# Meng-333/FastDiffSR

Measured on AMD Instinct MI355X. Metric: 256x256 SR images/sec at T=20, higher is better.
Workload: dtype f16x3; 1 GPU; x4 64->256, batch=16/GPU, T=20, random-init FastDiffSR UNet (inner 64, mults 1-2-4-4), 256x256, conv arithmetic f16x3 (BASELINE configs[1]); batch_per_gpu=16, global_batch=16, noise=drawn in the loop by the engine (Philox4x32-10), hipgraph=False, parallelism=dp1 (independent batches, weights broadcast once)

## Files before the change

### fastdiffsr_amd/_lib.py

```python
import ctypes as C
import os

from .build import LIB

FDSR_MAX_MULTS = 8
FDSR_SAMPLE_GRAPH = 1
FDSR_METRIC_FIELDS = 8
FDSR_SSIM_UNIFORM7, FDSR_SSIM_GAUSS11 = 1, 2
PRECISIONS = {'f32': 0, 'f16x3': 1, 'bf16': 2, 'f16': 3}


class FdsrConfig(C.Structure):
    _fields_ = [('in_channel', C.c_int32), ('out_channel', C.c_int32), ('inner_channel', C.c_int32),
                ('norm_groups', C.c_int32), ('n_mults', C.c_int32), ('channel_mults', C.c_int32 * FDSR_MAX_MULTS),
                ('res_blocks', C.c_int32), ('dropout', C.c_float), ('image_size', C.c_int32), ('variant', C.c_int32),
                ('n_attn_res', C.c_int32), ('attn_res', C.c_int32 * FDSR_MAX_MULTS)]


class FdsrSchedule(C.Structure):
    _fields_ = [('n_timestep', C.c_int32), ('noise_level', C.POINTER(C.c_float)), ('sqrt_recip', C.POINTER(C.c_float)),
                ('sqrt_recipm1', C.POINTER(C.c_float)), ('coef1', C.POINTER(C.c_float)), ('coef2', C.POINTER(C.c_float)),
                ('sigma', C.POINTER(C.c_float))]


# ... 15 lines not shown
class FdsrError(RuntimeError):
    def __init__(self, code, msg):
        super().__init__(f'libfdsr_hip error {code}: {msg}')
        self.code = code


class FdsrSaturated(FdsrError):
    """f16x3: a raw convolution input left the f16 range (FDSR_E_SATURATED): the call's output is not fp32-grade."""


FDSR_E_SATURATED = -6

K32 = {'F16X3': 1, 'BF16': 2, 'RIDER_16ROW': 4, 'SMALL_GRID_2ROW': 8, 'UP2': 16, 'SMALL_WG_F16X3': 32, 'SMALL_WG_RIDER_F16X3': 64,
       'SMALL_WG_BF16': 128, 'SMALL_WG_RIDER_BF16': 512, 'RIDER_FIRST_8WAVE': 1024}
K32_DEFAULT = 1 | 2 | 8 | 16 | 32 | 64 | 128 | 1024
STRIP = {'BF16_64': 1, 'F16X3_64': 2, 'BF16_ONE_WG': 4, 'BF16_CAT64': 8, 'BF16_RIDER': 16, 'BF16_CAT128': 32, 'BF16_COUT128': 64}
STRIP_DEFAULT = 1 | 2 | 8 | 16 | 64
STRIP_ALL = 127


def bit_names(table, value):
    return '|'.join(n for n, b in table.items() if value & b) or '0'


_lib = None

SYMBOLS = {
    'fdsr_create': (C.c_int, [C.POINTER(FdsrConfig), C.POINTER(C.c_void_p)]),
    'fdsr_destroy': (None, [C.c_void_p]),
    'fdsr_last_error': (C.c_char_p, [C.c_void_p]),
    'fdsr_version': (C.c_char_p, []),
    'fdsr_num_weights': (C.c_int, [C.c_void_p]),
    'fdsr_weight_info': (C.c_int, [C.c_void_p, C.c_int, C.c_char_p, C.c_int, C.POINTER(C.c_int64), C.POINTER(C.c_int),
# ... 120 lines not shown
```

### fastdiffsr_amd/csrc/fdsr_conv_strip.hip

```cpp
#include "fdsr_kernels.h"
#include "fdsr_act_io.h"

#include <type_traits>

namespace fdsr {

typedef float s_f32x4 __attribute__((ext_vector_type(4)));
typedef unsigned s_u32x4 __attribute__((ext_vector_type(4)));
typedef _Float16 s_h8 __attribute__((ext_vector_type(8)));
typedef __bf16 s_b8 __attribute__((ext_vector_type(8)));

template <int I, int N, class F>
__device__ __forceinline__ void static_for(F&& f) {
  if constexpr (I < N) {
    f(std::integral_constant<int, I>{});
    static_for<I + 1, N>(f);
  }
}

__device__ __forceinline__ float silu_s(float v) { return v * __builtin_amdgcn_rcpf(1.0f + __expf(-v)); }

#ifndef STRIP_XS
#define STRIP_XS 4
#endif
#ifndef STRIP_XS1
#define STRIP_XS1 4
#endif
#ifndef STRIP_DIAG
#define STRIP_DIAG 0
#endif
#ifndef STRIP_FENCE3
#define STRIP_FENCE3 1
#endif

template <int PREC, int C0_, int C1_, int CR0_, int CR1_, int NPH>
struct StripCfg {
  static constexpr int NP = PREC == PREC_F16X3 ? 2 : 1;
  static constexpr int ESZ = prec_is16(PREC) ? 2 : 4;
  static constexpr int WNP = PREC == PREC_BF16 ? 1 : 2;
  static constexpr int C0 = C0_, C1 = C1_, CIN = C0_ + C1_, KCH = CIN / 32, SW = 16 * NPH, HWD = SW + 2;
  static constexpr int OPP = CIN / 8;
  static constexpr int RB = 16 * OPP * NP;
  static constexpr int SLOT_BYTES = HWD * RB;
  static constexpr int NP0 = C0_ / 32, NP1 = C1_ / 32, NPM = NP0 + NP1;
  static constexpr int NF = 3 * KCH * NPH;
  static constexpr int CR0 = CR0_, CR1 = CR1_, CR = CR0_ + CR1_, KCR = CR / 32;
  static constexpr int RRB = CR * 2;
  static constexpr int RSLOT_BYTES = SW * RRB;
  static constexpr int NR0 = CR0_ / 32, NR1 = CR1_ / 32, NPR = NR0 + NR1;
  static constexpr int NFR = KCR * NPH;
  static constexpr int NT = NF + NFR;
  static constexpr int RSLOT_OFF = 2 * SLOT_BYTES;
  static constexpr int GTAB_OFF = RSLOT_OFF + 2 * RSLOT_BYTES;
  static constexpr int OSZ = prec_is16(PREC) ? 2 : 4;
  static constexpr int PB = 64 * OSZ;
  static constexpr int UPP = PB / 16;
  static constexpr int TILE_BYTES = SW * PB;
  static constexpr int OUT_OFF = GTAB_OFF + 64 * OPP;
  static constexpr int RES_OFF = OUT_OFF + 2 * TILE_BYTES;
  static constexpr int NIT = SW * PB / 16 / 256;
  static_assert(NPH == 4, "a staging pass = 32 channels of a 64-pixel row");
  static_assert(C0_ % 32 == 0 && C1_ % 32 == 0 && CR0_ % 32 == 0 && CR1_ % 32 == 0 && C0_ > 0, "whole 32-channel chunks");
  static_assert(256 % (C0_ / 8) == 0 && (C1_ == 0 || 256 % (C1_ / 8) == 0) && (CR0_ == 0 || 256 % (CR0_ / 8) == 0) &&
                (CR1_ == 0 || 256 % (CR1_ / 8) == 0), "a thread keeps one oct index per tensor");
  static_assert(RB == 128 || RB == 256 || RB == 384 || RB == 512, "swizzles below are verified for these pixel strides");
  static_assert(CR == 0 || (prec_is16(PREC) && (RRB == 256 || RRB == 384)), "riders: the 2-byte modes (f16: launched only while the rider and the main conv share one weight scale, conv_strip_ok)");
  static_assert(NIT >= 1 && NIT <= 4 && 256 % UPP == 0, "row-tile map");
  static_assert(SLOT_BYTES + 16 * (NPH - 1) * RB < 65536 && RSLOT_BYTES < 65536, "fragment offsets must fit the ds_read immediate");
  static constexpr int NITEMS = NIT + 5 * NPM + (C1_ ? 2 : 1) + NPR + 1;
  static constexpr int slot_of(int j) { return NPH + (j * (NT - NPH)) / NITEMS; }
  static constexpr int first_item(int f) {
    int j = 0;
    while (j < NITEMS && slot_of(j) < f) ++j;
    return j;
  }
};

template <int RB>
__device__ __forceinline__ int strip_swz(int px) {
  return (RB == 128 || RB == 384) ? 2 * ((px >> 1) & 3) : 2 * (px & 7);
}

template <int PREC> struct StripRaw;
template <> struct StripRaw<PREC_BF16> {
  uint4 v;
// ... 38 lines not shown
  unsigned v;
  __device__ __forceinline__ void load(const unsigned char* ptr) { v = *reinterpret_cast<const unsigned*>(ptr); }
  __device__ __forceinline__ void pair(float& a, float& b) const {
    typedef _Float16 h2t __attribute__((ext_vector_type(2)));
    const h2t h = __builtin_bit_cast(h2t, v);
    a = (float)h[0];
    b = (float)h[1];
  }
};
template <> struct StripRawPair<PREC_F16X3> {
  float2 v;
  __device__ __forceinline__ void load(const unsigned char* ptr) { v = *reinterpret_cast<const float2*>(ptr); }
  __device__ __forceinline__ void pair(float& a, float& b) const { a = v.x; b = v.y; }
};

template <int PREC, int C0_, int C1_, int CR0_, int CR1_, int NPH, bool HAS_RES, int LB>
__global__ void __launch_bounds__(256, LB) conv_strip_kernel(const ConvParams p, const int seg_rows, const int wn_a) {
  using Cfg = StripCfg<PREC, C0_, C1_, CR0_, CR1_, NPH>;
  constexpr int NP = Cfg::NP, RB = Cfg::RB, SW = Cfg::SW, OPP = Cfg::OPP, KCH = Cfg::KCH, NF = Cfg::NF, ESZ = Cfg::ESZ;
  constexpr int NP0 = Cfg::NP0, NP1 = Cfg::NP1, NPM = Cfg::NPM, KCR = Cfg::KCR, NPR = Cfg::NPR, NR0 = Cfg::NR0, NFR = Cfg::NFR, NT = Cfg::NT;
  constexpr int RRB = Cfg::RRB;
  constexpr bool CAT = C1_ > 0, RIDER = Cfg::CR > 0;
  constexpr int XS = (LB == 1 ? STRIP_XS1 : STRIP_XS) < NF ? (LB == 1 ? STRIP_XS1 : STRIP_XS) : NF;
  using IO = ActIO<PREC>;
  typedef typename IO::Quad Quad;

  extern __shared__ __attribute__((aligned(16))) unsigned char smem_s[];
  const int tid = threadIdx.x, lane = tid & 63, w = tid >> 6, c15 = lane & 15, g = lane >> 4;
  const int H = p.Hout, W = p.Wout;

  const int stripsX = W / SW, segs = (H + seg_rows - 1) / seg_rows;
  int bid;
  {
    const int nwg = gridDim.x, b = blockIdx.x;
    const int q8 = nwg >> 3, r8 = nwg & 7, xcd = b & 7, k = b >> 3;
    bid = (xcd < r8 ? xcd * (q8 + 1) : r8 * (q8 + 1) + (xcd - r8) * q8) + k;
  }
  const int ncg = p.Cout / 64;
  const int cg = bid % ncg;
  bid /= ncg;
  const int sx = bid % stripsX;
  bid /= stripsX;
  const int seg = bid % segs;
// ... 12 lines not shown
  } else { ot[1] = 0; ppx[1] = 0; og[1] = 0; tb[1] = tb[0]; }
  constexpr unsigned PIXB[2] = {C0_ * ESZ, (CAT ? C1_ : C0_) * ESZ};
  float* gtab = reinterpret_cast<float*>(smem_s + Cfg::GTAB_OFF);
  if (tid < 4 * OPP) {
    const int c = 8 * (tid >> 2) + 2 * (tid & 3);
    const float* ps = p.gn_scale + (size_t)n * Cfg::CIN + c;
    const float* ph = p.gn_shift + (size_t)n * Cfg::CIN + c;
    *reinterpret_cast<s_f32x4*>(gtab + 4 * tid) = s_f32x4{ps[0], ps[1], ph[0], ph[1]};
  }
  __syncthreads();
  int hdst[2];
  unsigned hcol[2];
  bool hok[2];
#pragma unroll
  for (int t = 0; t < (CAT ? 2 : 1); ++t) {
    const int hside = ((lane % (2 * OPPt[t])) / OPPt[t]) & 1;
    const int hix = hside ? ox0 + SW : ox0 - 1;
    hok[t] = hix >= 0 && hix < W;
    hcol[t] = (unsigned)(hok[t] ? hix : ox0) * PIXB[t] + 2 * w * ESZ;
    const int hpx = hside ? SW + 1 : 0;
    hdst[t] = hpx * RB + 16 * (og[t] ^ strip_swz<RB>(hpx)) + 4 * w;
  }

  StripRaw<PREC> raw[3][NPM];
  StripRawPair<PREC> rawh[3][CAT ? 2 : 1];
  s_u32x4 rraw[3][RIDER ? NPR : 1];
  auto crow_in = [&](int iy) __attribute__((always_inline)) {
    const int hi = oy1 < H - 1 ? oy1 : H - 1;
    return iy < 0 ? 0 : (iy > hi ? hi : iy);
  };
  auto load_pass = [&](int iy, StripRaw<PREC>* set, int q) __attribute__((always_inline)) {
    const int t = q < NP0 ? 0 : 1, i = q < NP0 ? q : q - NP0;
    set[q].load(tb[t] + ((unsigned)(crow_in(iy) * W) + (unsigned)(ox0 + ppx[t] + i * (256 / OPPt[t]))) * PIXB[t]);
  };
  auto load_halo = [&](int iy, StripRawPair<PREC>* set, int t) __attribute__((always_inline)) {
    set[t].load(tb[t] + ((unsigned)(crow_in(iy) * W) * PIXB[t] + hcol[t]));
  };
  constexpr int OPRt[2] = {RIDER ? CR0_ / 8 : 1, RIDER && CR1_ ? CR1_ / 8 : 1};
  const unsigned char* rb[2] = {nullptr, nullptr};
  int rdst[RIDER ? NPR : 1];
  unsigned rsrc[RIDER ? NPR : 1];
  if (RIDER) {
#pragma unroll
    for (int r = 0; r < NPR; ++r) {
      const int t = r < NR0 ? 0 : 1, i = r < NR0 ? r : r - NR0;
      const int o = tid % OPRt[t], px = tid / OPRt[t] + i * (256 / OPRt[t]);
      const int ogr = (t ? CR0_ / 8 : 0) + o;
      rdst[r] = px * RRB + 16 * (ogr ^ strip_swz<RRB>(px));
// ... 49 lines not shown
      act_s0(a, b, gtab + 16 * og[t] + 4 * k, atmp);
    }
    if (stage < 0 || stage == 1) act_s1(atmp);
    if (stage < 0 || stage == 2) act_s2(atmp, d.hi[k], d.lo[PREC == PREC_F16X3 ? k : 0]);
  };
  auto write_oct = [&](const Staged& d, bool ok, unsigned char* slot, int dofs) __attribute__((always_inline)) {
    const uint4 z = {0u, 0u, 0u, 0u};
    *reinterpret_cast<uint4*>(slot + dofs) = ok ? uint4{d.hi[0], d.hi[1], d.hi[2], d.hi[3]} : z;
    if (PREC == PREC_F16X3)
      *reinterpret_cast<uint4*>(slot + (dofs ^ (16 * OPP))) = ok ? uint4{d.lo[0], d.lo[1], d.lo[2], d.lo[3]} : z;
  };
  auto stage_halo = [&](const StripRawPair<PREC>& r, int t, bool ok, unsigned char* slot, int stage) __attribute__((always_inline)) {
    if (stage <= 0) {
      float a, b;
      r.pair(a, b);
      act_s0(a, b, gtab + 16 * og[t] + 4 * w, atmp);
    }
    if (stage < 0 || stage == 1) act_s1(atmp);
    if (stage < 0 || stage == 2) {
      unsigned hi, lo = 0;
      act_s2(atmp, hi, lo);
      *reinterpret_cast<unsigned*>(slot + hdst[t]) = ok ? hi : 0u;
      if (PREC == PREC_F16X3) *reinterpret_cast<unsigned*>(slot + (hdst[t] ^ (16 * OPP))) = ok ? lo : 0u;
    }
  };
  int pdst[NPM];
#pragma unroll
  for (int q = 0; q < NPM; ++q) {
    const int t = q < NP0 ? 0 : 1, i = q < NP0 ? q : q - NP0;
    const int px = 1 + ppx[t] + i * (256 / OPPt[t]);
    pdst[q] = px * RB + 16 * (og[t] ^ strip_swz<RB>(px));
  }
  Staged stg;

  uint4 Wf[3][3][KCH][NP];
  uint4 Wr[RIDER ? KCR : 1];
  {
    const uint4* wq = reinterpret_cast<const uint4*>(p.wq);
    const int nk16 = p.Cin_pad / 16, co32 = 2 * cg + (w >> 1), cot = co32 / wn_a, wna = co32 % wn_a;
    const int wlane = 32 * (g & 1) + 16 * (w & 1) + c15;
#pragma unroll
    for (int kc = 0; kc < KCH; ++kc)
#pragma unroll
      for (int tap = 0; tap < 9; ++tap) {
        const uint4* src = wq + ((((size_t)cot * nk16 + 2 * kc + (g >> 1)) * wn_a + wna) * 9 + tap) * (Cfg::WNP * 64) + wlane;
#pragma unroll
        for (int pl = 0; pl < NP; ++pl) Wf[tap / 3][tap % 3][kc][pl] = src[pl * 64];
      }
    if (RIDER) {
      const uint4* wr = reinterpret_cast<const uint4*>(p.wq_r);
#pragma unroll
      for (int kc = 0; kc < KCR; ++kc) Wr[kc] = wr[(((size_t)cot * p.nkr + 2 * kc + (g >> 1)) * wn_a + wna) * (Cfg::WNP * 64) + wlane];
    }
  }

  int xa[3][KCH][NP];
#pragma unroll
  for (int kx = 0; kx < 3; ++kx)
#pragma unroll
    for (int kc = 0; kc < KCH; ++kc)
#pragma unroll
      for (int pl = 0; pl < NP; ++pl) {
        const int px = c15 + kx;
        xa[kx][kc][pl] = px * RB + 16 * ((pl * OPP + 4 * kc + g) ^ strip_swz<RB>(px));
      }
  int xr[RIDER ? KCR : 1];
  if (RIDER) {
#pragma unroll
    for (int kc = 0; kc < KCR; ++kc) xr[kc] = c15 * RRB + 16 * ((4 * kc + g) ^ strip_swz<RRB>(c15));
  }

  s_f32x4 acc[3][NPH];
#pragma unroll
  for (int a = 0; a < 3; ++a)
#pragma unroll
    for (int ph = 0; ph < NPH; ++ph) acc[a][ph] = s_f32x4{0.f, 0.f, 0.f, 0.f};

  const int cob = 64 * cg + 16 * w + 4 * g;
  s_f32x4 add;
  {
    const float* tembp = p.temb ? p.temb + (size_t)n * p.temb_stride + p.temb_off : p.bias;
    const float tmul = p.temb ? 1.f : 0.f;
#pragma unroll
    for (int r = 0; r < 4; ++r) {
      float a = p.bias[cob + r];
      if (RIDER) a += p.bias_r[cob + r];
      add[r] = a + tmul * tembp[cob + r];
    }
  }
  const float winv = p.w_inv_scale_dev ? *p.w_inv_scale_dev : p.w_inv_scale;
  constexpr int OSZ = Cfg::OSZ, NIT = Cfg::NIT, TILE = Cfg::TILE_BYTES;
  s_f32x4 s1 = {0.f, 0.f, 0.f, 0.f}, s2 = {0.f, 0.f, 0.f, 0.f};
  unsigned char* otile = smem_s + Cfg::OUT_OFF;
  unsigned char* rtile = smem_s + Cfg::RES_OFF;
  constexpr int PB = Cfg::PB, UPP = Cfg::UPP;
  auto tsw = [](int px) { return OSZ == 2 ? ((px >> 1) & 7) : 2 * (px & 7); };
  const int aq = OSZ == 2 ? c15 * PB + 16 * (((4 * w + g) >> 1) ^ tsw(c15)) + 8 * (g & 1)
                          : c15 * PB + 16 * ((4 * w + g) ^ tsw(c15));
  const unsigned GPB = (unsigned)p.Cout * OSZ;
  int a128[NIT];
  unsigned gofs[NIT];
#pragma unroll
  for (int i = 0; i < NIT; ++i) {
    const int px = tid / UPP + (256 / UPP) * i, u = tid % UPP;
    a128[i] = px * PB + 16 * (u ^ tsw(px));
    gofs[i] = (unsigned)((ox0 + px) * GPB + 64 * cg * OSZ + 16 * u);
  }
  const size_t img = (size_t)n * H * W * GPB;
  unsigned char* outn = reinterpret_cast<unsigned char*>(p.out) + img;
  const unsigned char* resn = reinterpret_cast<const unsigned char*>(HAS_RES ? p.res : p.out) + img;
  const uint4 z4 = {0u, 0u, 0u, 0u};
  uint4 rres0 = z4, rres1 = z4, rres2 = z4, rres3 = z4;
  auto crow = [&](int oy) __attribute__((always_inline)) { return oy < oy0 ? oy0 : (oy >= oy1 ? oy1 - 1 : oy); };
  auto load_res = [&](int oy) __attribute__((always_inline)) {
    if (HAS_RES && !(STRIP_DIAG & 1)) {
      const unsigned r0 = (unsigned)(crow(oy) * W) * GPB;
      rres0 = *reinterpret_cast<const uint4*>(resn + (r0 + gofs[0]));
      if (NIT > 1) rres1 = *reinterpret_cast<const uint4*>(resn + (r0 + gofs[NIT > 1 ? 1 : 0]));
      if (NIT > 2) rres2 = *reinterpret_cast<const uint4*>(resn + (r0 + gofs[NIT > 2 ? 2 : 0]));
// ... 13 lines not shown
    s_f32x4 v = a * winv + add;
    if (HAS_RES) v += IO::widen(*reinterpret_cast<const Quad*>(rtile + (oy & 1) * TILE + aq + 16 * PB * ph));
    unsigned char* dst = otile + (oy & 1) * TILE + aq + 16 * PB * ph;
    if (OSZ == 2) {
      *reinterpret_cast<uint2*>(dst) = pack4_16<PREC>(v);
    } else {
      *reinterpret_cast<s_f32x4*>(dst) = v;
    }
    s1 += v;
    s2 += v * v;
  };
  auto flush = [&](int oy, int i) __attribute__((always_inline)) {
    const uint4 v = *reinterpret_cast<const uint4*>(otile + (oy & 1) * TILE + a128[i]);
    if (!(STRIP_DIAG & 2)) *reinterpret_cast<uint4*>(outn + ((unsigned)(oy * W) * GPB + gofs[i])) = v;
  };

  uint4 Xf[XS][NP];
  auto mfma1 = [&](const uint4* wf, const uint4* xf, s_f32x4 c) __attribute__((always_inline)) -> s_f32x4 {
    if (PREC == PREC_F16X3) {
      c = __builtin_amdgcn_mfma_f32_16x16x32_f16(__builtin_bit_cast(s_h8, wf[0]), __builtin_bit_cast(s_h8, xf[NP - 1]), c, 0, 0, 0);
      c = __builtin_amdgcn_mfma_f32_16x16x32_f16(__builtin_bit_cast(s_h8, wf[NP - 1]), __builtin_bit_cast(s_h8, xf[0]), c, 0, 0, 0);
      return __builtin_amdgcn_mfma_f32_16x16x32_f16(__builtin_bit_cast(s_h8, wf[0]), __builtin_bit_cast(s_h8, xf[0]), c, 0, 0, 0);
    }
    return mfma16_k32<PREC>(wf[0], xf[0], c);
  };
  auto step = [&](int iy, int it, auto rot_tag, auto epi_tag, auto flush_tag) __attribute__((always_inline)) {
    constexpr int ROT = decltype(rot_tag)::value;
    constexpr bool EPI = decltype(epi_tag)::value, FLUSH = decltype(flush_tag)::value;
    constexpr int A0 = (ROT + 1) % 3, A1 = ROT, A2 = (ROT + 2) % 3;
    StripRaw<PREC>* rset = raw[(ROT + 1) % 3];
    StripRawPair<PREC>* hset = rawh[(ROT + 1) % 3];
    s_u32x4* rrs = rraw[(ROT + 1) % 3];
    unsigned char* cur = smem_s + (it & 1) * Cfg::SLOT_BYTES;
    unsigned char* nxt = smem_s + ((it & 1) ^ 1) * Cfg::SLOT_BYTES;
    unsigned char* rcur = smem_s + Cfg::RSLOT_OFF + (it & 1) * Cfg::RSLOT_BYTES;
    unsigned char* rnxt = smem_s + Cfg::RSLOT_OFF + ((it & 1) ^ 1) * Cfg::RSLOT_BYTES;
    const bool rok = iy + 1 >= 0 && iy + 1 < H;
    auto load_x = [&](auto fc) __attribute__((always_inline)) {
      constexpr int f = decltype(fc)::value;
      if constexpr (f < NF) {
        constexpr int ph = f % NPH, kc = (f / NPH) % KCH, kx = f / (NPH * KCH);
#pragma unroll
        for (int pl = 0; pl < NP; ++pl)
          Xf[f % XS][pl] = *reinterpret_cast<const uint4*>(cur + xa[kx][kc][pl] + ph * 16 * RB);
      } else if constexpr (f < NT) {
        constexpr int ph = (f - NF) % NPH, kc = (f - NF) / NPH;
        Xf[f % XS][0] = *reinterpret_cast<const uint4*>(rcur + xr[kc] + ph * 16 * RRB);
      }
    };
    auto item = [&](auto jc, auto sc) __attribute__((always_inline)) {
      constexpr int j = decltype(jc)::value, stage = decltype(sc)::value;
      constexpr int J1 = NIT, J2 = J1 + 5 * NPM, J3 = J2 + (CAT ? 2 : 1), J4 = J3 + NPR;
      constexpr bool last = stage < 0 || stage == 2;
      if constexpr (j < J1) {
        if (FLUSH && last) flush(iy - 3, j);
      } else if constexpr (j < J2) {
// ... 6 lines not shown
      } else if constexpr (j < J3) {
        constexpr int t = j - J2;
        stage_halo(hset[t], t, hok[t] && rok, nxt, stage);
        if constexpr (last) load_halo(iy + 4, hset, t);
      } else if constexpr (j < J4) {
        constexpr int r = j - J3;
        if constexpr (last) {
          *reinterpret_cast<s_u32x4*>(rnxt + rdst[r]) = rrs[r];
          load_rider(iy + 4, rrs, r);
        }
      } else if constexpr (last) {
        res_to_lds(iy - 1);
        load_res(iy);
      }
    };
    static_for<0, XS - 1>(load_x);
    static_for<0, NT>([&](auto fc) __attribute__((always_inline)) {
      constexpr int f = decltype(fc)::value;
      load_x(std::integral_constant<int, f + XS - 1>{});
      if constexpr (EPI && f < NPH) finish(iy - 2, f, acc[A0][f]);
      constexpr int J0 = Cfg::first_item(f), J1e = Cfg::first_item(f + 1);
      static_assert(J1e - J0 <= 1, "one item per slot (the activation stages share one set of temporaries)");
      typedef std::integral_constant<int, 0> S0;
      typedef std::integral_constant<int, 1> S1;
      typedef std::integral_constant<int, 2> S2;
      typedef std::integral_constant<int, -1> SA;
      if constexpr (f < NF) {
        constexpr int ph = f % NPH, kc = (f / NPH) % KCH, kx = f / (NPH * KCH);
        constexpr bool fresh = kx == 0 && kc == 0;
        const s_f32x4 zero = {0.f, 0.f, 0.f, 0.f};
        acc[A2][ph] = mfma1(Wf[2][kx][kc], Xf[f % XS], acc[A2][ph]);
        static_for<J0, J1e>([&](auto jc) __attribute__((always_inline)) { item(jc, S0{}); });
        if (STRIP_FENCE3) __builtin_amdgcn_sched_barrier(0);
        acc[A1][ph] = mfma1(Wf[1][kx][kc], Xf[f % XS], acc[A1][ph]);
        static_for<J0, J1e>([&](auto jc) __attribute__((always_inline)) { item(jc, S1{}); });
        if (STRIP_FENCE3) __builtin_amdgcn_sched_barrier(0);
        acc[A0][ph] = mfma1(Wf[0][kx][kc], Xf[f % XS], fresh ? zero : acc[A0][ph]);
        static_for<J0, J1e>([&](auto jc) __attribute__((always_inline)) { item(jc, S2{}); });
      } else {
        constexpr int ph = (f - NF) % NPH, kc = (f - NF) / NPH;
        acc[A1][ph] = mfma16_k32<PREC>(Wr[kc], Xf[f % XS][0], acc[A1][ph]);
        static_for<J0, J1e>([&](auto jc) __attribute__((always_inline)) { item(jc, SA{}); });
      }
      __builtin_amdgcn_sched_barrier(0);
    });
    __syncthreads();
  };
  typedef std::integral_constant<int, 0> R0;
  typedef std::integral_constant<int, 1> R1;
  typedef std::integral_constant<int, 2> R2;

  {
    StripRaw<PREC> first[NPM];
    StripRawPair<PREC> firsth[CAT ? 2 : 1];
    s_u32x4 firstr[RIDER ? NPR : 1];
#pragma unroll
    for (int q = 0; q < NPM; ++q) load_pass(oy0 - 1, first, q);
#pragma unroll
    for (int t = 0; t < (CAT ? 2 : 1); ++t) load_halo(oy0 - 1, firsth, t);
    if (RIDER) {
// ... 29 lines not shown
  const int nsteps = oy1 - oy0 + 2;
  load_res(oy0);
  step(oy0 - 1, 0, R0{}, std::false_type{}, std::false_type{});
  step(oy0, 1, R1{}, std::false_type{}, std::false_type{});
  step(oy0 + 1, 2, R2{}, std::false_type{}, std::false_type{});
  step(oy0 + 2, 3, R0{}, std::true_type{}, std::false_type{});
  for (int it = 4; it < nsteps; it += 3) {
    step(oy0 - 1 + it, it, R1{}, std::true_type{}, std::true_type{});
    if (it + 1 < nsteps) step(oy0 + it, it + 1, R2{}, std::true_type{}, std::true_type{});
    if (it + 2 < nsteps) step(oy0 + 1 + it, it + 2, R0{}, std::true_type{}, std::true_type{});
  }
#pragma unroll
  for (int i = 0; i < NIT; ++i) flush(oy1 - 2, i);
  {
    const int last = ((nsteps - 1) % 3 + 2) % 3;
#pragma unroll
    for (int q = 0; q < NPH; ++q) finish(oy1 - 1, q, last == 0 ? acc[0][q] : (last == 1 ? acc[1][q] : acc[2][q]));
  }
  __syncthreads();
#pragma unroll
  for (int i = 0; i < NIT; ++i) flush(oy1 - 1, i);

  if (p.part_out) {
    float vals[8] = {s1[0], s2[0], s1[1], s2[1], s1[2], s2[2], s1[3], s2[3]};
#pragma unroll
    for (int e = 0; e < 8; ++e)
#pragma unroll
      for (int m = 8; m >= 1; m >>= 1) vals[e] += __shfl_xor(vals[e], m, 64);
    if (c15 == 0) {
      float* dst = p.part_out + (((size_t)n * (segs * stripsX) + seg * stripsX + sx) * p.Cout + cob) * 2;
      *reinterpret_cast<s_f32x4*>(dst) = s_f32x4{vals[0], vals[1], vals[2], vals[3]};
      *reinterpret_cast<s_f32x4*>(dst + 4) = s_f32x4{vals[4], vals[5], vals[6], vals[7]};
    }
  }
}

#ifndef STRIP_PART
#define STRIP_PART 0
#endif
#define STRIP_INSTANCES_F16X3(X) X(PREC_F16X3, 64, 0, 0, 0, false, 1) X(PREC_F16X3, 64, 0, 0, 0, true, 1)
#define STRIP_INSTANCES_16(X, P)                                                                                  \
  X(P, 64, 0, 0, 0, false, 2) X(P, 64, 0, 0, 0, true, 2) X(P, 64, 0, 0, 0, false, 1) X(P, 64, 0, 0, 0, true, 1)      \
  X(P, 64, 64, 0, 0, false, 1) X(P, 128, 64, 0, 0, false, 1) X(P, 64, 0, 64, 64, false, 1) X(P, 64, 0, 128, 64, false, 1) \
  X(P, 128, 0, 0, 0, false, 1) X(P, 128, 0, 0, 0, true, 1)
#define STRIP_DEFINE(P, A, B, C, D, R, L) template __global__ void conv_strip_kernel<P, A, B, C, D, 4, R, L>(const ConvParams, const int, const int);
#define STRIP_DECLARE(P, A, B, C, D, R, L) extern template __global__ void conv_strip_kernel<P, A, B, C, D, 4, R, L>(const ConvParams, const int, const int);
#if STRIP_PART == 2
STRIP_INSTANCES_16(STRIP_DEFINE, PREC_BF16)
#elif STRIP_PART == 3
STRIP_INSTANCES_16(STRIP_DEFINE, PREC_F16)
#else
STRIP_INSTANCES_16(STRIP_DECLARE, PREC_BF16)
STRIP_INSTANCES_16(STRIP_DECLARE, PREC_F16)
#endif

// ... 20 lines not shown
    shape = prec_is16(prec) && (g_tun.strip & FDSR_STRIP_BF16_COUT128) && !p.xr0 && p.C1 == 0 && (p.C0 == 64 || p.C0 == 128);
  } else if (p.xr0) {
    if (prec == PREC_F16 && p.w_inv_scale > 0.f && p.w_inv_scale_r > 0.f && p.w_inv_scale_r != p.w_inv_scale) return false;
    shape = prec_is16(prec) && (g_tun.strip & FDSR_STRIP_BF16_RIDER) && !p.res && p.C0 == 64 && p.C1 == 0 && p.Cr1 == 64 && (p.Cr0 == 64 || p.Cr0 == 128) &&
            p.nkr * 16 == p.Cr0 + p.Cr1;
  } else if (p.C1) {
    shape = prec_is16(prec) && !p.res && p.C1 == 64 && ((p.C0 == 64 && (g_tun.strip & FDSR_STRIP_BF16_CAT64)) || (p.C0 == 128 && (g_tun.strip & FDSR_STRIP_BF16_CAT128)));
  } else {
    shape = p.C0 == 64 && (g_tun.strip & (prec_is16(prec) ? FDSR_STRIP_BF16_64 : FDSR_STRIP_F16X3_64));
  }
  if (!shape) return false;
  const long wgs = (long)p.N * ((p.Wout + 63) / 64) * ((p.Hout + 15) / 16) * (p.Cout / 64);
  return wgs >= strip_min_wgs(p, prec);
}

template <int PREC, int C0_, int C1_, int CR0_, int CR1_, bool HAS_RES, int LB>
static hipError_t launch_strip_t(const ConvParams& p, int wn_a, hipStream_t s, int* tiles) {
  using Cfg = StripCfg<PREC, C0_, C1_, CR0_, CR1_, 4>;
  const int rows = strip_seg_rows(p, Cfg::SW, PREC);
  const int stripsX = (p.Wout + Cfg::SW - 1) / Cfg::SW, segs = (p.Hout + rows - 1) / rows;
  if (tiles) *tiles = stripsX * segs;
  const size_t lds = (size_t)Cfg::RES_OFF + (HAS_RES ? 2 * Cfg::TILE_BYTES : 0);
  hipLaunchKernelGGL((conv_strip_kernel<PREC, C0_, C1_, CR0_, CR1_, 4, HAS_RES, LB>), dim3(p.N * stripsX * segs * (p.Cout / 64)), dim3(256), lds, s, p, rows, wn_a);
  return hipGetLastError();
}

hipError_t launch_conv_strip(int prec, const ConvParams& p, int wn_a, hipStream_t s, int* tiles) {
  if (prec == PREC_F16X3) {
    return p.res ? launch_strip_t<PREC_F16X3, 64, 0, 0, 0, true, 1>(p, wn_a, s, tiles) : launch_strip_t<PREC_F16X3, 64, 0, 0, 0, false, 1>(p, wn_a, s, tiles);
  }
  if (prec == PREC_F16) {
    if (p.xr0)
      return p.Cr0 == 64 ? launch_strip_t<PREC_F16, 64, 0, 64, 64, false, 1>(p, wn_a, s, tiles) : launch_strip_t<PREC_F16, 64, 0, 128, 64, false, 1>(p, wn_a, s, tiles);
    if (p.C0 == 128 && !p.C1)
      return p.res ? launch_strip_t<PREC_F16, 128, 0, 0, 0, true, 1>(p, wn_a, s, tiles) : launch_strip_t<PREC_F16, 128, 0, 0, 0, false, 1>(p, wn_a, s, tiles);
    if (p.C1)
      return p.C0 == 64 ? launch_strip_t<PREC_F16, 64, 64, 0, 0, false, 1>(p, wn_a, s, tiles) : launch_strip_t<PREC_F16, 128, 64, 0, 0, false, 1>(p, wn_a, s, tiles);
    if (g_tun.strip & FDSR_STRIP_BF16_ONE_WG)
      return p.res ? launch_strip_t<PREC_F16, 64, 0, 0, 0, true, 1>(p, wn_a, s, tiles) : launch_strip_t<PREC_F16, 64, 0, 0, 0, false, 1>(p, wn_a, s, tiles);
    return p.res ? launch_strip_t<PREC_F16, 64, 0, 0, 0, true, 2>(p, wn_a, s, tiles) : launch_strip_t<PREC_F16, 64, 0, 0, 0, false, 2>(p, wn_a, s, tiles);
  }
  if (prec != PREC_BF16) return hipErrorInvalidValue;
  if (p.C0 == 128 && !p.C1)
    return p.res ? launch_strip_t<PREC_BF16, 128, 0, 0, 0, true, 1>(p, wn_a, s, tiles) : launch_strip_t<PREC_BF16, 128, 0, 0, 0, false, 1>(p, wn_a, s, tiles);
  if (p.xr0) {
    return p.Cr0 == 64 ? launch_strip_t<PREC_BF16, 64, 0, 64, 64, false, 1>(p, wn_a, s, tiles) : launch_strip_t<PREC_BF16, 64, 0, 128, 64, false, 1>(p, wn_a, s, tiles);
  }
  if (p.C1) {
    return p.C0 == 64 ? launch_strip_t<PREC_BF16, 64, 64, 0, 0, false, 1>(p, wn_a, s, tiles) : launch_strip_t<PREC_BF16, 128, 64, 0, 0, false, 1>(p, wn_a, s, tiles);
  }
  if (g_tun.strip & FDSR_STRIP_BF16_ONE_WG)
    return p.res ? launch_strip_t<PREC_BF16, 64, 0, 0, 0, true, 1>(p, wn_a, s, tiles) : launch_strip_t<PREC_BF16, 64, 0, 0, 0, false, 1>(p, wn_a, s, tiles);
  return p.res ? launch_strip_t<PREC_BF16, 64, 0, 0, 0, true, 2>(p, wn_a, s, tiles) : launch_strip_t<PREC_BF16, 64, 0, 0, 0, false, 2>(p, wn_a, s, tiles);
}

template <int PREC, int C0_, int C1_, int CR0_, int CR1_, bool HAS_RES, int LB>
static hipError_t init_strip_t() {
  return hipFuncSetAttribute(reinterpret_cast<const void*>(conv_strip_kernel<PREC, C0_, C1_, CR0_, CR1_, 4, HAS_RES, LB>),
                             hipFuncAttributeMaxDynamicSharedMemorySize, 160 * 1024);
}

hipError_t kernels_strip_init() {
  hipError_t e;
#define X(P, A, B, C, D, R, L) if ((e = init_strip_t<P, A, B, C, D, R, L>()) != hipSuccess) return e;
  STRIP_INSTANCES_F16X3(X)
  STRIP_INSTANCES_16(X, PREC_BF16)
  STRIP_INSTANCES_16(X, PREC_F16)
#undef X
  return hipSuccess;
}
#endif

}
```

### include/fdsr.h

```cpp
#ifndef FDSR_H_
#define FDSR_H_

#include <stddef.h>
#include <stdint.h>

#ifdef __cplusplus
extern "C" {
#endif

#define FDSR_OK 0
#define FDSR_E_INVALID (-1)
#define FDSR_E_KEY (-2)
#define FDSR_E_STATE (-3)
#define FDSR_E_WORKSPACE (-4)
#define FDSR_E_HIP (-5)
#define FDSR_E_SATURATED (-6)

#define FDSR_MAX_MULTS 8

typedef struct fdsr_engine* fdsr_handle;

typedef struct fdsr_config {
  int32_t in_channel;
  int32_t out_channel;
// ... 164 lines not shown
  FDSR_K32_SMALL_WG_F16X3 = 32,
  FDSR_K32_SMALL_WG_RIDER_F16X3 = 64,
  FDSR_K32_SMALL_WG_BF16 = 128,
  FDSR_K32_SMALL_WG_RIDER_BF16 = 512,
  FDSR_K32_RIDER_FIRST_8WAVE = 1024,
  FDSR_K32_DEFAULT = 1 | 2 | 8 | 16 | 32 | 64 | 128 | 1024
};
enum fdsr_strip_bits {
  FDSR_STRIP_BF16_64 = 1,
  FDSR_STRIP_F16X3_64 = 2,
  FDSR_STRIP_BF16_ONE_WG = 4,
  FDSR_STRIP_BF16_CAT64 = 8,
  FDSR_STRIP_BF16_RIDER = 16,
  FDSR_STRIP_BF16_CAT128 = 32,
  FDSR_STRIP_BF16_COUT128 = 64,
  FDSR_STRIP_DEFAULT = 1 | 2 | 8 | 16 | 64
};

int fdsr_debug_option(const char* name, long long value);
int fdsr_set_debug(fdsr_handle h, int on);
int fdsr_debug_tensor(fdsr_handle h, const char* name, const float** dev_ptr,
                      int* n, int* hgt, int* wid, int* ch);
int fdsr_debug_tensor_elem_bytes(fdsr_handle h, const char* name, int* bytes);
int fdsr_profile_begin(fdsr_handle h);
int fdsr_profile_end(fdsr_handle h, int* launches, double* conv_ms, double* conv_flops,
                     double* conv_bytes);

int fdsr_set_training(fdsr_handle h, int on);
int fdsr_set_dropout_seed(fdsr_handle h, uint64_t seed);
int fdsr_debug_dropout_mask(fdsr_handle h, const char* block, const unsigned char** dev_off, int* n, int* hgt, int* wid,
                            int* ch, float* scale);
// ... 28 lines not shown
```

Measured before the change: 73.69 images/s.

## Split f16x3 strip conv K-dimension across wave pairs with LDS reduction

Adds a wave-pair form of the f16x3 strip convolution: workgroups of 512 threads, where two wave groups each take half of the input-channel chunks and exchange partial accumulators through double-buffered LDS before the epilogue. Each wave then finishes half of the pixel phases, and the partial-sum statistics are reduced across halves as well. The aim is to halve the per-wave weight register footprint so two workgroups fit per CU (launch bound 2), raising occupancy for the 64-channel f16x3 convs. It adds LDS exchange traffic, and the extra barriers and cross-wave dependencies could offset the gain. The new form is enabled by default through a new strip flag.

```diff
diff --git a/fastdiffsr_amd/_lib.py b/fastdiffsr_amd/_lib.py
--- a/fastdiffsr_amd/_lib.py
+++ b/fastdiffsr_amd/_lib.py
@@ -53,9 +53,9 @@
 K32 = {'F16X3': 1, 'BF16': 2, 'RIDER_16ROW': 4, 'SMALL_GRID_2ROW': 8, 'UP2': 16, 'SMALL_WG_F16X3': 32, 'SMALL_WG_RIDER_F16X3': 64,
        'SMALL_WG_BF16': 128, 'SMALL_WG_RIDER_BF16': 512, 'RIDER_FIRST_8WAVE': 1024}
 K32_DEFAULT = 1 | 2 | 8 | 16 | 32 | 64 | 128 | 1024
-STRIP = {'BF16_64': 1, 'F16X3_64': 2, 'BF16_ONE_WG': 4, 'BF16_CAT64': 8, 'BF16_RIDER': 16, 'BF16_CAT128': 32, 'BF16_COUT128': 64}
-STRIP_DEFAULT = 1 | 2 | 8 | 16 | 64
-STRIP_ALL = 127
+STRIP = {'BF16_64': 1, 'F16X3_64': 2, 'BF16_ONE_WG': 4, 'BF16_CAT64': 8, 'BF16_RIDER': 16, 'BF16_CAT128': 32, 'BF16_COUT128': 64, 'F16X3_PAIR': 128}
+STRIP_DEFAULT = 1 | 2 | 8 | 16 | 64 | 128
+STRIP_ALL = 255
 
 
 def bit_names(table, value):
diff --git a/fastdiffsr_amd/csrc/fdsr_conv_strip.hip b/fastdiffsr_amd/csrc/fdsr_conv_strip.hip
--- a/fastdiffsr_amd/csrc/fdsr_conv_strip.hip
+++ b/fastdiffsr_amd/csrc/fdsr_conv_strip.hip
@@ -25,6 +25,9 @@
 #endif
 #ifndef STRIP_XS1
 #define STRIP_XS1 4
+#endif
+#ifndef STRIP_XSP
+#define STRIP_XSP 2
 #endif
 #ifndef STRIP_DIAG
 #define STRIP_DIAG 0
@@ -33,8 +36,10 @@
 #define STRIP_FENCE3 1
 #endif
 
-template <int PREC, int C0_, int C1_, int CR0_, int CR1_, int NPH>
+template <int PREC, int C0_, int C1_, int CR0_, int CR1_, int NPH, int KS = 1>
 struct StripCfg {
+  static constexpr int NTHR = 256 * KS;
+  static constexpr int NEPI = NPH / KS;
   static constexpr int NP = PREC == PREC_F16X3 ? 2 : 1;
   static constexpr int ESZ = prec_is16(PREC) ? 2 : 4;
   static constexpr int WNP = PREC == PREC_BF16 ? 1 : 2;
@@ -42,8 +47,9 @@
   static constexpr int OPP = CIN / 8;
   static constexpr int RB = 16 * OPP * NP;
   static constexpr int SLOT_BYTES = HWD * RB;
-  static constexpr int NP0 = C0_ / 32, NP1 = C1_ / 32, NPM = NP0 + NP1;
-  static constexpr int NF = 3 * KCH * NPH;
+  static constexpr int NP0 = C0_ / (32 * KS), NP1 = C1_ / (32 * KS), NPM = NP0 + NP1;
+  static constexpr int KCW = KCH / KS;
+  static constexpr int NF = 3 * KCW * NPH;
   static constexpr int CR0 = CR0_, CR1 = CR1_, CR = CR0_ + CR1_, KCR = CR / 32;
   static constexpr int RRB = CR * 2;
   static constexpr int RSLOT_BYTES = SW * RRB;
@@ -56,19 +62,22 @@
   static constexpr int PB = 64 * OSZ;
   static constexpr int UPP = PB / 16;
   static constexpr int TILE_BYTES = SW * PB;
-  static constexpr int OUT_OFF = GTAB_OFF + 64 * OPP;
+  static constexpr int XCH_OFF = GTAB_OFF + 64 * OPP;
+  static constexpr int XCH_BYTES = KS > 1 ? 4 * KS * NEPI * 64 * 16 : 0;
+  static constexpr int OUT_OFF = XCH_OFF + 2 * XCH_BYTES;
   static constexpr int RES_OFF = OUT_OFF + 2 * TILE_BYTES;
-  static constexpr int NIT = SW * PB / 16 / 256;
+  static constexpr int NIT = SW * PB / 16 / NTHR;
   static_assert(NPH == 4, "a staging pass = 32 channels of a 64-pixel row");
-  static_assert(C0_ % 32 == 0 && C1_ % 32 == 0 && CR0_ % 32 == 0 && CR1_ % 32 == 0 && C0_ > 0, "whole 32-channel chunks");
-  static_assert(256 % (C0_ / 8) == 0 && (C1_ == 0 || 256 % (C1_ / 8) == 0) && (CR0_ == 0 || 256 % (CR0_ / 8) == 0) &&
+  static_assert(C0_ % (32 * KS) == 0 && C1_ % (32 * KS) == 0 && CR0_ % 32 == 0 && CR1_ % 32 == 0 && C0_ > 0, "whole 32-channel chunks, whole staging passes");
+  static_assert(NTHR % (C0_ / 8) == 0 && (C1_ == 0 || NTHR % (C1_ / 8) == 0) && (CR0_ == 0 || 256 % (CR0_ / 8) == 0) &&
                 (CR1_ == 0 || 256 % (CR1_ / 8) == 0), "a thread keeps one oct index per tensor");
+  static_assert(KS == 1 || (KS == 2 && NEPI == 2 && PREC == PREC_F16X3 && CR0_ + CR1_ == 0), "the wave-pair form: f16x3 without a rider");
   static_assert(RB == 128 || RB == 256 || RB == 384 || RB == 512, "swizzles below are verified for these pixel strides");
   static_assert(CR == 0 || (prec_is16(PREC) && (RRB == 256 || RRB == 384)), "riders: the 2-byte modes (f16: launched only while the rider and the main conv share one weight scale, conv_strip_ok)");
-  static_assert(NIT >= 1 && NIT <= 4 && 256 % UPP == 0, "row-tile map");
+  static_assert(NIT >= 1 && NIT <= 4 && NTHR % UPP == 0, "row-tile map");
   static_assert(SLOT_BYTES + 16 * (NPH - 1) * RB < 65536 && RSLOT_BYTES < 65536, "fragment offsets must fit the ds_read immediate");
   static constexpr int NITEMS = NIT + 5 * NPM + (C1_ ? 2 : 1) + NPR + 1;
-  static constexpr int slot_of(int j) { return NPH + (j * (NT - NPH)) / NITEMS; }
+  static constexpr int slot_of(int j) { return NEPI + (j * (NT - NEPI)) / NITEMS; }
   static constexpr int first_item(int f) {
     int j = 0;
     while (j < NITEMS && slot_of(j) < f) ++j;
@@ -137,19 +146,22 @@
   __device__ __forceinline__ void pair(float& a, float& b) const { a = v.x; b = v.y; }
 };
 
-template <int PREC, int C0_, int C1_, int CR0_, int CR1_, int NPH, bool HAS_RES, int LB>
-__global__ void __launch_bounds__(256, LB) conv_strip_kernel(const ConvParams p, const int seg_rows, const int wn_a) {
-  using Cfg = StripCfg<PREC, C0_, C1_, CR0_, CR1_, NPH>;
-  constexpr int NP = Cfg::NP, RB = Cfg::RB, SW = Cfg::SW, OPP = Cfg::OPP, KCH = Cfg::KCH, NF = Cfg::NF, ESZ = Cfg::ESZ;
+template <int PREC, int C0_, int C1_, int CR0_, int CR1_, int NPH, bool HAS_RES, int LB, int KS = 1>
+__global__ void __launch_bounds__(256 * KS, LB) conv_strip_kernel(const ConvParams p, const int seg_rows, const int wn_a) {
+  using Cfg = StripCfg<PREC, C0_, C1_, CR0_, CR1_, NPH, KS>;
+  constexpr int NP = Cfg::NP, RB = Cfg::RB, SW = Cfg::SW, OPP = Cfg::OPP, KCW = Cfg::KCW, NF = Cfg::NF, ESZ = Cfg::ESZ;
+  constexpr int NTHR = Cfg::NTHR, NEPI = Cfg::NEPI;
   constexpr int NP0 = Cfg::NP0, NP1 = Cfg::NP1, NPM = Cfg::NPM, KCR = Cfg::KCR, NPR = Cfg::NPR, NR0 = Cfg::NR0, NFR = Cfg::NFR, NT = Cfg::NT;
   constexpr int RRB = Cfg::RRB;
   constexpr bool CAT = C1_ > 0, RIDER = Cfg::CR > 0;
-  constexpr int XS = (LB == 1 ? STRIP_XS1 : STRIP_XS) < NF ? (LB == 1 ? STRIP_XS1 : STRIP_XS) : NF;
+  constexpr int XS0 = KS > 1 ? STRIP_XSP : (LB == 1 ? STRIP_XS1 : STRIP_XS), XS = XS0 < NF ? XS0 : NF;
   using IO = ActIO<PREC>;
   typedef typename IO::Quad Quad;
 
   extern __shared__ __attribute__((aligned(16))) unsigned char smem_s[];
-  const int tid = threadIdx.x, lane = tid & 63, w = tid >> 6, c15 = lane & 15, g = lane >> 4;
+  const int tid = threadIdx.x, lane = tid & 63, c15 = lane & 15, g = lane >> 4;
+  const int w = KS > 1 ? __builtin_amdgcn_readfirstlane(tid >> 6) : tid >> 6;
+  const int wc = w & 3, h = KS > 1 ? w >> 2 : 0;
   const int H = p.Hout, W = p.Wout;
 
   const int stripsX = W / SW, segs = (H + seg_rows - 1) / seg_rows;
@@ -192,12 +204,12 @@
   bool hok[2];
 #pragma unroll
   for (int t = 0; t < (CAT ? 2 : 1); ++t) {
-    const int hside = ((lane % (2 * OPPt[t])) / OPPt[t]) & 1;
+    const int hside = KS > 1 ? h : ((lane % (2 * OPPt[t])) / OPPt[t]) & 1;
     const int hix = hside ? ox0 + SW : ox0 - 1;
     hok[t] = hix >= 0 && hix < W;
-    hcol[t] = (unsigned)(hok[t] ? hix : ox0) * PIXB[t] + 2 * w * ESZ;
+    hcol[t] = (unsigned)(hok[t] ? hix : ox0) * PIXB[t] + 2 * wc * ESZ;
     const int hpx = hside ? SW + 1 : 0;
-    hdst[t] = hpx * RB + 16 * (og[t] ^ strip_swz<RB>(hpx)) + 4 * w;
+    hdst[t] = hpx * RB + 16 * (og[t] ^ strip_swz<RB>(hpx)) + 4 * wc;
   }
 
   StripRaw<PREC> raw[3][NPM];
@@ -209,7 +221,7 @@
   };
   auto load_pass = [&](int iy, StripRaw<PREC>* set, int q) __attribute__((always_inline)) {
     const int t = q < NP0 ? 0 : 1, i = q < NP0 ? q : q - NP0;
-    set[q].load(tb[t] + ((unsigned)(crow_in(iy) * W) + (unsigned)(ox0 + ppx[t] + i * (256 / OPPt[t]))) * PIXB[t]);
+    set[q].load(tb[t] + ((unsigned)(crow_in(iy) * W) + (unsigned)(ox0 + ppx[t] + i * (NTHR / OPPt[t]))) * PIXB[t]);
   };
   auto load_halo = [&](int iy, StripRawPair<PREC>* set, int t) __attribute__((always_inline)) {
     set[t].load(tb[t] + ((unsigned)(crow_in(iy) * W) * PIXB[t] + hcol[t]));
@@ -289,7 +301,7 @@
     if (stage <= 0) {
       float a, b;
       r.pair(a, b);
-      act_s0(a, b, gtab + 16 * og[t] + 4 * w, atmp);
+      act_s0(a, b, gtab + 16 * og[t] + 4 * wc, atmp);
     }
     if (stage < 0 || stage == 1) act_s1(atmp);
     if (stage < 0 || stage == 2) {
@@ -303,24 +315,24 @@
 #pragma unroll
   for (int q = 0; q < NPM; ++q) {
     const int t = q < NP0 ? 0 : 1, i = q < NP0 ? q : q - NP0;
-    const int px = 1 + ppx[t] + i * (256 / OPPt[t]);
+    const int px = 1 + ppx[t] + i * (NTHR / OPPt[t]);
     pdst[q] = px * RB + 16 * (og[t] ^ strip_swz<RB>(px));
   }
   Staged stg;
 
-  uint4 Wf[3][3][KCH][NP];
+  uint4 Wf[3][3][KCW][NP];
   uint4 Wr[RIDER ? KCR : 1];
   {
     const uint4* wq = reinterpret_cast<const uint4*>(p.wq);
-    const int nk16 = p.Cin_pad / 16, co32 = 2 * cg + (w >> 1), cot = co32 / wn_a, wna = co32 % wn_a;
-    const int wlane = 32 * (g & 1) + 16 * (w & 1) + c15;
-#pragma unroll
-    for (int kc = 0; kc < KCH; ++kc)
+    const int nk16 = p.Cin_pad / 16, co32 = 2 * cg + (wc >> 1), cot = co32 / wn_a, wna = co32 % wn_a;
+    const int wlane = 32 * (g & 1) + 16 * (wc & 1) + c15;
+#pragma unroll
+    for (int kcl = 0; kcl < KCW; ++kcl)
 #pragma unroll
       for (int tap = 0; tap < 9; ++tap) {
-        const uint4* src = wq + ((((size_t)cot * nk16 + 2 * kc + (g >> 1)) * wn_a + wna) * 9 + tap) * (Cfg::WNP * 64) + wlane;
-#pragma unroll
-        for (int pl = 0; pl < NP; ++pl) Wf[tap / 3][tap % 3][kc][pl] = src[pl * 64];
+        const uint4* src = wq + ((((size_t)cot * nk16 + 2 * (KS * kcl + h) + (g >> 1)) * wn_a + wna) * 9 + tap) * (Cfg::WNP * 64) + wlane;
+#pragma unroll
+        for (int pl = 0; pl < NP; ++pl) Wf[tap / 3][tap % 3][kcl][pl] = src[pl * 64];
       }
     if (RIDER) {
       const uint4* wr = reinterpret_cast<const uint4*>(p.wq_r);
@@ -329,15 +341,15 @@
     }
   }
 
-  int xa[3][KCH][NP];
+  int xa[3][KCW][NP];
 #pragma unroll
   for (int kx = 0; kx < 3; ++kx)
 #pragma unroll
-    for (int kc = 0; kc < KCH; ++kc)
+    for (int kcl = 0; kcl < KCW; ++kcl)
 #pragma unroll
       for (int pl = 0; pl < NP; ++pl) {
         const int px = c15 + kx;
-        xa[kx][kc][pl] = px * RB + 16 * ((pl * OPP + 4 * kc + g) ^ strip_swz<RB>(px));
+        xa[kx][kcl][pl] = px * RB + 16 * ((pl * OPP + 4 * (KS * kcl + h) + g) ^ strip_swz<RB>(px));
       }
   int xr[RIDER ? KCR : 1];
   if (RIDER) {
@@ -351,7 +363,7 @@
 #pragma unroll
     for (int ph = 0; ph < NPH; ++ph) acc[a][ph] = s_f32x4{0.f, 0.f, 0.f, 0.f};
 
-  const int cob = 64 * cg + 16 * w + 4 * g;
+  const int cob = 64 * cg + 16 * wc + 4 * g;
   s_f32x4 add;
   {
     const float* tembp = p.temb ? p.temb + (size_t)n * p.temb_stride + p.temb_off : p.bias;
@@ -370,14 +382,14 @@
   unsigned char* rtile = smem_s + Cfg::RES_OFF;
   constexpr int PB = Cfg::PB, UPP = Cfg::UPP;
   auto tsw = [](int px) { return OSZ == 2 ? ((px >> 1) & 7) : 2 * (px & 7); };
-  const int aq = OSZ == 2 ? c15 * PB + 16 * (((4 * w + g) >> 1) ^ tsw(c15)) + 8 * (g & 1)
-                          : c15 * PB + 16 * ((4 * w + g) ^ tsw(c15));
+  const int aq = OSZ == 2 ? c15 * PB + 16 * (((4 * wc + g) >> 1) ^ tsw(c15)) + 8 * (g & 1)
+                          : c15 * PB + 16 * ((4 * wc + g) ^ tsw(c15));
   const unsigned GPB = (unsigned)p.Cout * OSZ;
   int a128[NIT];
   unsigned gofs[NIT];
 #pragma unroll
   for (int i = 0; i < NIT; ++i) {
-    const int px = tid / UPP + (256 / UPP) * i, u = tid % UPP;
+    const int px = tid / UPP + (NTHR / UPP) * i, u = tid % UPP;
     a128[i] = px * PB + 16 * (u ^ tsw(px));
     gofs[i] = (unsigned)((ox0 + px) * GPB + 64 * cg * OSZ + 16 * u);
   }
@@ -421,6 +433,20 @@
     const uint4 v = *reinterpret_cast<const uint4*>(otile + (oy & 1) * TILE + a128[i]);
     if (!(STRIP_DIAG & 2)) *reinterpret_cast<uint4*>(outn + ((unsigned)(oy * W) * GPB + gofs[i])) = v;
   };
+
+  unsigned char* xch = smem_s + Cfg::XCH_OFF;
+  const int xwr = (w * NEPI * 64 + lane) * 16, xrd = ((w ^ 4) * NEPI * 64 + lane) * 16;
+  auto half_pick = [&](s_f32x4 a0, s_f32x4 a1) __attribute__((always_inline)) -> s_f32x4 {
+    asm("" : "+v"(a0), "+v"(a1));
+    return h ? a1 : a0;
+  };
+  auto xch_send = [&](int area, int q, s_f32x4 lo, s_f32x4 hi) __attribute__((always_inline)) {
+    *reinterpret_cast<s_f32x4*>(xch + area * Cfg::XCH_BYTES + xwr + q * 1024) = half_pick(hi, lo);
+  };
+  auto xch_recv = [&](int area, int q) __attribute__((always_inline)) -> s_f32x4 {
+    return *reinterpret_cast<const s_f32x4*>(xch + area * Cfg::XCH_BYTES + xrd + q * 1024);
+  };
+  auto pair_sum = [&](s_f32x4 lo, s_f32x4 hi, s_f32x4 other) __attribute__((always_inline)) -> s_f32x4 { return half_pick(lo, hi) + other; };
 
   uint4 Xf[XS][NP];
   auto mfma1 = [&](const uint4* wf, const uint4* xf, s_f32x4 c) __attribute__((always_inline)) -> s_f32x4 {
@@ -446,7 +472,7 @@
     auto load_x = [&](auto fc) __attribute__((always_inline)) {
       constexpr int f = decltype(fc)::value;
       if constexpr (f < NF) {
-        constexpr int ph = f % NPH, kc = (f / NPH) % KCH, kx = f / (NPH * KCH);
+        constexpr int ph = f % NPH, kc = (f / NPH) % KCW, kx = f / (NPH * KCW);
 #pragma unroll
         for (int pl = 0; pl < NP; ++pl)
           Xf[f % XS][pl] = *reinterpret_cast<const uint4*>(cur + xa[kx][kc][pl] + ph * 16 * RB);
@@ -483,11 +509,19 @@
         load_res(iy);
       }
     };
+    s_f32x4 xin0, xin1;
+    if constexpr (KS > 1 && EPI) {
+      xin0 = xch_recv((it & 1) ^ 1, 0);
+      xin1 = xch_recv((it & 1) ^ 1, 1);
+    }
     static_for<0, XS - 1>(load_x);
     static_for<0, NT>([&](auto fc) __attribute__((always_inline)) {
       constexpr int f = decltype(fc)::value;
       load_x(std::integral_constant<int, f + XS - 1>{});
-      if constexpr (EPI && f < NPH) finish(iy - 2, f, acc[A0][f]);
+      if constexpr (EPI && f < NEPI) {
+        if constexpr (KS > 1) finish(iy - 2, NEPI * h + f, pair_sum(acc[A0][f], acc[A0][f + NEPI], f == 0 ? xin0 : xin1));
+        else finish(iy - 2, f, acc[A0][f]);
+      }
       constexpr int J0 = Cfg::first_item(f), J1e = Cfg::first_item(f + 1);
       static_assert(J1e - J0 <= 1, "one item per slot (the activation stages share one set of temporaries)");
       typedef std::integral_constant<int, 0> S0;
@@ -495,7 +529,7 @@
       typedef std::integral_constant<int, 2> S2;
       typedef std::integral_constant<int, -1> SA;
       if constexpr (f < NF) {
-        constexpr int ph = f % NPH, kc = (f / NPH) % KCH, kx = f / (NPH * KCH);
+        constexpr int ph = f % NPH, kc = (f / NPH) % KCW, kx = f / (NPH * KCW);
         constexpr bool fresh = kx == 0 && kc == 0;
         const s_f32x4 zero = {0.f, 0.f, 0.f, 0.f};
         acc[A2][ph] = mfma1(Wf[2][kx][kc], Xf[f % XS], acc[A2][ph]);
@@ -513,6 +547,12 @@
       }
       __builtin_amdgcn_sched_barrier(0);
     });
+    if constexpr (KS > 1) {
+      static_for<0, NEPI>([&](auto qc) __attribute__((always_inline)) {
+        constexpr int q = decltype(qc)::value;
+        xch_send(it & 1, q, acc[A2][q], acc[A2][q + NEPI]);
+      });
+    }
     __syncthreads();
   };
   typedef std::integral_constant<int, 0> R0;
@@ -572,8 +612,17 @@
   for (int i = 0; i < NIT; ++i) flush(oy1 - 2, i);
   {
     const int last = ((nsteps - 1) % 3 + 2) % 3;
-#pragma unroll
-    for (int q = 0; q < NPH; ++q) finish(oy1 - 1, q, last == 0 ? acc[0][q] : (last == 1 ? acc[1][q] : acc[2][q]));
+    if constexpr (KS > 1) {
+      static_for<0, NEPI>([&](auto qc) __attribute__((always_inline)) {
+        constexpr int q = decltype(qc)::value;
+        s_f32x4 m0 = half_pick(acc[0][q], acc[0][q + NEPI]), m1 = half_pick(acc[1][q], acc[1][q + NEPI]), m2 = half_pick(acc[2][q], acc[2][q + NEPI]);
+        asm("" : "+v"(m0), "+v"(m1), "+v"(m2));
+        finish(oy1 - 1, NEPI * h + q, (last == 0 ? m0 : (last == 1 ? m1 : m2)) + xch_recv((nsteps - 1) & 1, q));
+      });
+    } else {
+#pragma unroll
+      for (int q = 0; q < NPH; ++q) finish(oy1 - 1, q, last == 0 ? acc[0][q] : (last == 1 ? acc[1][q] : acc[2][q]));
+    }
   }
   __syncthreads();
 #pragma unroll
@@ -585,7 +634,18 @@
     for (int e = 0; e < 8; ++e)
 #pragma unroll
       for (int m = 8; m >= 1; m >>= 1) vals[e] += __shfl_xor(vals[e], m, 64);
-    if (c15 == 0) {
+    if constexpr (KS > 1) {
+      float* px = reinterpret_cast<float*>(xch) + 8 * (4 * wc + g);
+      if (h == 1 && c15 == 0) {
+        *reinterpret_cast<s_f32x4*>(px) = s_f32x4{vals[0], vals[1], vals[2], vals[3]};
+        *reinterpret_cast<s_f32x4*>(px + 4) = s_f32x4{vals[4], vals[5], vals[6], vals[7]};
+      }
+      __syncthreads();
+      const s_f32x4 o0 = *reinterpret_cast<const s_f32x4*>(px), o1 = *reinterpret_cast<const s_f32x4*>(px + 4);
+#pragma unroll
+      for (int e = 0; e < 4; ++e) { vals[e] += o0[e]; vals[4 + e] += o1[e]; }
+    }
+    if (c15 == 0 && h == 0) {
       float* dst = p.part_out + (((size_t)n * (segs * stripsX) + seg * stripsX + sx) * p.Cout + cob) * 2;
       *reinterpret_cast<s_f32x4*>(dst) = s_f32x4{vals[0], vals[1], vals[2], vals[3]};
       *reinterpret_cast<s_f32x4*>(dst + 4) = s_f32x4{vals[4], vals[5], vals[6], vals[7]};
@@ -597,6 +657,7 @@
 #define STRIP_PART 0
 #endif
 #define STRIP_INSTANCES_F16X3(X) X(PREC_F16X3, 64, 0, 0, 0, false, 1) X(PREC_F16X3, 64, 0, 0, 0, true, 1)
+#define STRIP_INSTANCES_F16X3_PAIR(X) X(PREC_F16X3, 64, 0, false) X(PREC_F16X3, 64, 0, true)
 #define STRIP_INSTANCES_16(X, P)                                                                                  \
   X(P, 64, 0, 0, 0, false, 2) X(P, 64, 0, 0, 0, true, 2) X(P, 64, 0, 0, 0, false, 1) X(P, 64, 0, 0, 0, true, 1)      \
   X(P, 64, 64, 0, 0, false, 1) X(P, 128, 64, 0, 0, false, 1) X(P, 64, 0, 64, 64, false, 1) X(P, 64, 0, 128, 64, false, 1) \
@@ -647,19 +708,22 @@
   return wgs >= strip_min_wgs(p, prec);
 }
 
-template <int PREC, int C0_, int C1_, int CR0_, int CR1_, bool HAS_RES, int LB>
+template <int PREC, int C0_, int C1_, int CR0_, int CR1_, bool HAS_RES, int LB, int KS = 1>
 static hipError_t launch_strip_t(const ConvParams& p, int wn_a, hipStream_t s, int* tiles) {
-  using Cfg = StripCfg<PREC, C0_, C1_, CR0_, CR1_, 4>;
+  using Cfg = StripCfg<PREC, C0_, C1_, CR0_, CR1_, 4, KS>;
   const int rows = strip_seg_rows(p, Cfg::SW, PREC);
   const int stripsX = (p.Wout + Cfg::SW - 1) / Cfg::SW, segs = (p.Hout + rows - 1) / rows;
   if (tiles) *tiles = stripsX * segs;
   const size_t lds = (size_t)Cfg::RES_OFF + (HAS_RES ? 2 * Cfg::TILE_BYTES : 0);
-  hipLaunchKernelGGL((conv_strip_kernel<PREC, C0_, C1_, CR0_, CR1_, 4, HAS_RES, LB>), dim3(p.N * stripsX * segs * (p.Cout / 64)), dim3(256), lds, s, p, rows, wn_a);
+  static_assert(Cfg::RES_OFF + 2 * Cfg::TILE_BYTES <= 160 * 1024, "LDS of one workgroup");
+  hipLaunchKernelGGL((conv_strip_kernel<PREC, C0_, C1_, CR0_, CR1_, 4, HAS_RES, LB, KS>), dim3(p.N * stripsX * segs * (p.Cout / 64)), dim3(Cfg::NTHR), lds, s, p, rows, wn_a);
   return hipGetLastError();
 }
 
 hipError_t launch_conv_strip(int prec, const ConvParams& p, int wn_a, hipStream_t s, int* tiles) {
   if (prec == PREC_F16X3) {
+    if (g_tun.strip & FDSR_STRIP_F16X3_PAIR)
+      return p.res ? launch_strip_t<PREC_F16X3, 64, 0, 0, 0, true, 2, 2>(p, wn_a, s, tiles) : launch_strip_t<PREC_F16X3, 64, 0, 0, 0, false, 2, 2>(p, wn_a, s, tiles);
     return p.res ? launch_strip_t<PREC_F16X3, 64, 0, 0, 0, true, 1>(p, wn_a, s, tiles) : launch_strip_t<PREC_F16X3, 64, 0, 0, 0, false, 1>(p, wn_a, s, tiles);
   }
   if (prec == PREC_F16) {
@@ -687,9 +751,9 @@
   return p.res ? launch_strip_t<PREC_BF16, 64, 0, 0, 0, true, 2>(p, wn_a, s, tiles) : launch_strip_t<PREC_BF16, 64, 0, 0, 0, false, 2>(p, wn_a, s, tiles);
 }
 
-template <int PREC, int C0_, int C1_, int CR0_, int CR1_, bool HAS_RES, int LB>
+template <int PREC, int C0_, int C1_, int CR0_, int CR1_, bool HAS_RES, int LB, int KS = 1>
 static hipError_t init_strip_t() {
-  return hipFuncSetAttribute(reinterpret_cast<const void*>(conv_strip_kernel<PREC, C0_, C1_, CR0_, CR1_, 4, HAS_RES, LB>),
+  return hipFuncSetAttribute(reinterpret_cast<const void*>(conv_strip_kernel<PREC, C0_, C1_, CR0_, CR1_, 4, HAS_RES, LB, KS>),
                              hipFuncAttributeMaxDynamicSharedMemorySize, 160 * 1024);
 }
 
@@ -700,6 +764,9 @@
   STRIP_INSTANCES_16(X, PREC_BF16)
   STRIP_INSTANCES_16(X, PREC_F16)
 #undef X
+#define X(P, A, B, R) if ((e = init_strip_t<P, A, B, 0, 0, R, 2, 2>()) != hipSuccess) return e;
+  STRIP_INSTANCES_F16X3_PAIR(X)
+#undef X
   return hipSuccess;
 }
 #endif
diff --git a/include/fdsr.h b/include/fdsr.h
--- a/include/fdsr.h
+++ b/include/fdsr.h
@@ -202,7 +202,8 @@
   FDSR_STRIP_BF16_RIDER = 16,
   FDSR_STRIP_BF16_CAT128 = 32,
   FDSR_STRIP_BF16_COUT128 = 64,
-  FDSR_STRIP_DEFAULT = 1 | 2 | 8 | 16 | 64
+  FDSR_STRIP_F16X3_PAIR = 128,
+  FDSR_STRIP_DEFAULT = 1 | 2 | 8 | 16 | 64 | 128
 };
 
 int fdsr_debug_option(const char* name, long long value);
```

Measured after the change: 73.81 images/s (median of 6 runs). About the same (+0.2%).
